# sunjay/portrayer

Hardware: AMD Instinct MI355X
Metric: Mray/s (primary+shadow+secondary) at 1920x1080 SAMPLES=64 (higher is better)
Workload: dtype f64; 1 GPU; big-scene (1000 analytic primitives, 3 point lights, reference scene script) 1920x1080 SAMPLES=64; width=1920, height=1080, samples=64, traversal=flat, sampling=counter-based jitter, seed 0, partition=single GPU, rays_per_frame=367740795

## Files before the change

### include/portrayer_hip.h

```cpp
#ifndef PORTRAYER_HIP_H
#define PORTRAYER_HIP_H

#include <stdint.h>

#ifdef __cplusplus
extern "C" {
#endif

#define PT_ABI_VERSION 8

enum { PT_PRIM_SPHERE = 0, PT_PRIM_TRIANGLE = 1, PT_PRIM_MESH = 2, PT_PRIM_KDMESH = 3, PT_PRIM_PLANE = 4, PT_PRIM_CUBE = 5, PT_PRIM_CYLINDER = 6, PT_PRIM_CONE = 7 };
enum { PT_TRAVERSE_FLAT = 1, PT_TRAVERSE_KD = 2, PT_TRAVERSE_HIER = 3 };
enum { PT_SAMPLE_CENTRE = 0, PT_SAMPLE_RNG = 1 };

enum {
    PT_OK = 0,
    PT_ERR_ARGUMENT = -1,
    PT_ERR_DEVICE = -2,
    PT_ERR_NO_SCENE = -3,
    PT_ERR_SLICE = -4,
    PT_ERR_SCENE = -5,
    PT_ERR_TRAVERSAL = -6
};

// ... 370 lines not shown
int pt_test_scene_info(const pt_context *ctx, uint64_t out[4]);
int pt_test_vertex_box_shape(const pt_context *ctx, uint64_t out[2]);
int pt_test_math(pt_context *ctx, int op, uint64_t n, const double *a, const double *b, double *out);
int pt_test_pow_host(uint64_t n, const double *x, const double *y, double *port, double *libm);
int pt_test_libm_host(int op, uint64_t n, const double *a, const double *b, double *out);
int pt_test_work_items(const pt_render_params *params, uint32_t *sample_count, uint64_t *sample_index_sum, uint32_t *chunk_length_sum,
                       uint64_t *n_items, uint32_t *lane_pixels_chunks_samples);
typedef struct pt_scene_traits {
    int32_t traverse;
    uint32_t n_nodes, n_lights;
    int32_t has_meshes;
    int32_t has_kdmesh;
    int32_t reflective;
    int32_t reflective_opaque;
    int32_t glossy;
    int32_t area_light;
    int32_t pad;
    uint64_t instanced_tris;
} pt_scene_traits;
int pt_test_kernel_choice(const pt_scene_traits *traits, int mode, int textured, uint32_t *kernel_mode, uint32_t *kernel_variant);
int pt_test_raypk(uint64_t n, int body, const double *origins, const double *directions, const double *t_max, const float *box_lo, const float *box_hi,
                  int32_t *verdict, float *t_near, float *t_far);
int pt_test_certain_shadow(uint64_t n, int type, const double *fwd, const double *inv, const double *P, const double *L, int32_t *out_certain, int32_t *out_exact_hit);
int pt_test_pixel_beam(uint64_t n, const double *cameras, const uint32_t *pixels, const double *jitters, const float *box_lo, const float *box_hi,
                       int32_t *accept, float *bound, int32_t *walk, double *rays);
int pt_test_pixel_list_summary(pt_context *ctx, uint64_t *out);
int pt_test_rect_beam(uint64_t n, const double *cameras, const uint32_t *rects, const double *offsets, const float *box_lo, const float *box_hi,
                      int32_t *accept, float *bound, int32_t *walk, double *rays);
int pt_test_pixel_list_records(pt_context *ctx, uint32_t *out, uint64_t words, uint64_t *info);
int pt_test_film_fold_host(uint32_t n, const double *samples, const uint32_t *cuts, uint32_t n_cuts, double out_sum[3]);
int pt_test_film_moments_host(uint32_t n, const double *samples, const uint32_t *cuts, uint32_t n_cuts, double out_sum[3], double *out_q, double *out_err);
int pt_test_film_plan_host(uint32_t width, uint32_t height, const pt_rect *slice, const uint32_t *budget, uint32_t max_samples, uint32_t round, uint32_t *list, uint32_t cap,
                           uint32_t *n_out);
int pt_test_film_plan(pt_context *ctx, uint32_t width, uint32_t height, const pt_rect *slice, const uint32_t *budget, uint32_t max_samples, uint32_t round, uint32_t *list, uint32_t cap,
                      uint32_t *n_out);
int pt_test_denoise_host(uint32_t width, uint32_t height, const pt_denoise_params *params, const double *linear, const double *variance, const uint32_t *counts,
                         const pt_denoise_guides *guides, double *out_linear, double *out_variance);
int pt_test_denoise_albedo_host(uint32_t width, uint32_t height, const pt_denoise_params *params, const double *linear, const double *variance, const uint32_t *counts,
                                const pt_denoise_guides *guides, const double *albedo, double *out_linear, double *out_variance);

#ifdef __cplusplus
}
#endif
#endif
```

### portrayer_amd/_hip.py

```python
from __future__ import annotations

import ctypes as C
import os
from typing import Optional

import numpy as np

PKG_DIR = os.path.dirname(os.path.abspath(__file__))
LIB_PATH = os.path.join(PKG_DIR, "libportrayer_hip.so")

TRAVERSE_FLAT, TRAVERSE_KD, TRAVERSE_HIER = 1, 2, 3
SAMPLE_CENTRE, SAMPLE_RNG = 0, 1
OK, ERR_ARGUMENT, ERR_DEVICE, ERR_NO_SCENE, ERR_SLICE, ERR_SCENE, ERR_TRAVERSAL = 0, -1, -2, -3, -4, -5, -6
KERNEL_WAVES_MASK, KERNEL_INTERPRETER, KERNEL_PARK, KERNEL_COUNTING, KERNEL_TEXTURED, KERNEL_FORK, KERNEL_CHAIN = 15, 16, 32, 64, 128, 256, 512

_dp = C.POINTER(C.c_double)
_ip = C.POINTER(C.c_int32)
_up = C.POINTER(C.c_uint32)
_u64p = C.POINTER(C.c_uint64)
_u8p = C.POINTER(C.c_uint8)


class PortrayerHipError(RuntimeError):
    pass
# ... 173 lines not shown

class PtStats(C.Structure):
    _fields_ = [(n, C.c_uint64) for n in ("primary", "shadow", "reflect", "refract", "depth11_skipped", "hits", "n_inner", "n_leaf",
                                          "n_analytic", "n_tri", "n_bbox", "kd_plane_miss", "stack_overflow")] + \
               [("kernel_ms", C.c_double), ("total_ms", C.c_double), ("diag", C.c_uint64 * 8), ("kernel_mode", C.c_uint32), ("kernel_variant", C.c_uint32)]

    def as_dict(self):
        d = {n: (float if n.endswith("_ms") else int)(getattr(self, n)) for n, _ in self._fields_ if n != "diag"}
        d["diag"] = [int(x) for x in self.diag]
        return d


_lib: Optional[C.CDLL] = None

EXPORTS = ["pt_abi_version", "pt_device_count", "pt_context_create", "pt_context_destroy", "pt_last_error", "pt_scene_upload",
           "pt_render", "pt_render_device", "pt_render_finish", "pt_context_stream", "pt_context_next_slot", "pt_compact_bytes", "pt_untile_device", "pt_tile_slot_pixel", "pt_untile_host", "pt_device_alloc",
           "pt_device_free", "pt_copy_to_device", "pt_copy_from_device", "pt_synchronize", "pt_measure_copy_bandwidth", "pt_test_cast_rays",
           "pt_test_math", "pt_test_work_items", "pt_node_create", "pt_node_destroy", "pt_node_last_error", "pt_node_ranks", "pt_node_uses_rccl", "pt_node_context",
           "pt_node_scene_upload", "pt_node_render", "pt_node_upload_background", "pt_node_render_resident", "pt_node_download_image",
           "pt_node_device", "pt_node_frame_begin", "pt_node_frame_end", "pt_node_frames_in_flight", "pt_node_last_frame_host_ms", "pt_node_last_frame_rank_kernel_ms", "pt_test_pow_host", "pt_test_libm_host",
           "pt_aov", "pt_aov_device", "pt_aov_finish", "pt_rays", "pt_rays_device", "pt_rays_finish", "pt_segments", "pt_segments_device",
           "pt_radiance", "pt_radiance_device", "pt_radiance_finish", "pt_scene_update", "pt_node_scene_update", "pt_scene_deform", "pt_node_scene_deform", "pt_scene_mesh_rebuildable", "pt_test_scene_bytes", "pt_test_scene_info",
           "pt_vertex_bounds_device", "pt_scene_deform_device", "pt_test_vertex_box_shape", "pt_test_raypk", "pt_test_certain_shadow", "pt_test_pixel_beam", "pt_test_pixel_list_summary", "pt_test_rect_beam", "pt_test_pixel_list_records",
           "pt_film_create", "pt_film_destroy", "pt_film_reset", "pt_film_add", "pt_film_add_device", "pt_film_resolve", "pt_film_resolve_device", "pt_film_counts",
           "pt_test_film_fold_host",
           "pt_film_create_moments", "pt_film_add_map", "pt_film_add_map_device", "pt_film_error", "pt_film_error_device", "pt_film_budget_device",
           "pt_test_film_moments_host", "pt_test_film_plan_host", "pt_test_film_plan",
           "pt_film_denoise", "pt_film_denoise_device", "pt_test_denoise_host",
           "pt_guides", "pt_guides_device", "pt_guides_finish", "pt_film_denoise_albedo", "pt_film_denoise_albedo_device", "pt_test_denoise_albedo_host",
           "pt_ao", "pt_ao_device", "pt_ao_finish", "pt_test_ao_rays_host", "pt_test_ao_tables",
           "pt_gather", "pt_gather_device", "pt_gather_finish", "pt_test_kernel_choice",
           "pt_chart_triangles", "pt_chart", "pt_chart_device", "pt_test_chart_host",
           "pt_direct", "pt_direct_device", "pt_direct_finish", "pt_test_direct_host"]


def header_functions():
    import re
    with open(os.path.join(os.path.dirname(os.path.dirname(os.path.abspath(__file__))), "include", "portrayer_hip.h")) as fh:
        text = re.sub(r"/\*.*?\*/", "", fh.read(), flags=re.S)
    return sorted(set(re.findall(r"\b(pt_[a-z0-9_]+)\s*\(", text)))


def missing_symbols():
    l = lib()
    return [n for n in header_functions() if not hasattr(l, n)]

# ... 50 lines not shown
        l.pt_untile_device.argtypes = [C.c_void_p, C.POINTER(PtRenderParams), C.c_void_p, C.c_void_p, C.c_void_p]
        l.pt_tile_slot_pixel.restype = C.c_int
        l.pt_tile_slot_pixel.argtypes = [C.POINTER(PtRenderParams), C.c_uint32, C.c_uint32, _up, _up]
        l.pt_untile_host.restype = C.c_int
        l.pt_untile_host.argtypes = [C.POINTER(PtRenderParams), _u8p, _u8p]
        l.pt_device_alloc.restype = C.c_int
        l.pt_device_alloc.argtypes = [C.c_void_p, C.c_uint64, C.POINTER(C.c_void_p)]
        l.pt_device_free.restype = C.c_int
        l.pt_device_free.argtypes = [C.c_void_p, C.c_void_p]
        l.pt_copy_to_device.restype = C.c_int
        l.pt_copy_to_device.argtypes = [C.c_void_p, C.c_void_p, C.c_void_p, C.c_uint64]
        l.pt_copy_from_device.restype = C.c_int
        l.pt_copy_from_device.argtypes = [C.c_void_p, C.c_void_p, C.c_void_p, C.c_uint64]
        l.pt_synchronize.restype = C.c_int
        l.pt_synchronize.argtypes = [C.c_void_p]
        l.pt_measure_copy_bandwidth.restype = C.c_int
        l.pt_measure_copy_bandwidth.argtypes = [C.c_void_p, C.c_uint64, C.c_int, _dp]
        l.pt_test_cast_rays.restype = C.c_int
        l.pt_test_cast_rays.argtypes = [C.c_void_p, C.c_uint64, _dp, _dp, C.c_int, _dp, _ip, _ip]
        l.pt_test_work_items.restype = C.c_int
        l.pt_test_work_items.argtypes = [C.c_void_p, C.POINTER(C.c_uint32), C.POINTER(C.c_uint64), C.POINTER(C.c_uint32), C.POINTER(C.c_uint64), C.POINTER(C.c_uint32)]
        l.pt_test_certain_shadow.restype = C.c_int
        l.pt_test_certain_shadow.argtypes = [C.c_uint64, C.c_int, _dp, _dp, _dp, _dp, _ip, _ip]
        l.pt_test_raypk.restype = C.c_int
        l.pt_test_raypk.argtypes = [C.c_uint64, C.c_int, _dp, _dp, _dp, C.POINTER(C.c_float), C.POINTER(C.c_float), _ip, C.POINTER(C.c_float), C.POINTER(C.c_float)]
        l.pt_test_pixel_list_summary.restype = C.c_int
        l.pt_test_pixel_list_summary.argtypes = [C.c_void_p, C.POINTER(C.c_uint64)]
        l.pt_test_pixel_beam.restype = C.c_int
        l.pt_test_pixel_beam.argtypes = [C.c_uint64, _dp, C.POINTER(C.c_uint32), _dp, C.POINTER(C.c_float), C.POINTER(C.c_float), _ip, C.POINTER(C.c_float), _ip, _dp]
        l.pt_test_rect_beam.restype = C.c_int
        l.pt_test_rect_beam.argtypes = l.pt_test_pixel_beam.argtypes
        l.pt_test_pixel_list_records.restype = C.c_int
        l.pt_test_pixel_list_records.argtypes = [C.c_void_p, C.POINTER(C.c_uint32), C.c_uint64, C.POINTER(C.c_uint64)]
        l.pt_test_math.restype = C.c_int
        l.pt_test_math.argtypes = [C.c_void_p, C.c_int, C.c_uint64, _dp, _dp, _dp]
        l.pt_node_create.restype = C.c_int
        l.pt_node_create.argtypes = [C.c_int, _ip, C.POINTER(C.c_void_p)]
        l.pt_node_destroy.restype = None
        l.pt_node_destroy.argtypes = [C.c_void_p]
        l.pt_node_last_error.restype = C.c_char_p
        l.pt_node_last_error.argtypes = [C.c_void_p]
        l.pt_node_ranks.restype = C.c_int
        l.pt_node_ranks.argtypes = [C.c_void_p]
        l.pt_node_uses_rccl.restype = C.c_int
        l.pt_node_uses_rccl.argtypes = [C.c_void_p]
        l.pt_node_context.restype = C.c_void_p
# ... 215 lines not shown
```

### portrayer_amd/csrc/pt_api.hip

```cpp
#include <type_traits>

#include "pt_context.h"
#include "pt_aov_inst.h"
#include "pt_guides_inst.h"
#include "pt_chart.h"
#include "pt_rays_inst.h"
#include "pt_segments_inst.h"
#include "pt_ao_inst.h"
#include "pt_direct_inst.h"
#include "pt_radiance_inst.h"
#include "pt_gather_inst.h"
#include "pt_film_inst.h"
#include "pt_film_map_inst.h"
#include "pt_denoise.h"
#include "pt_render_inst.h"
#include "pt_shade.h"
#include "pt_pixel_list.h"

template <int MODE>
__global__ void __launch_bounds__(PT_BLOCK) pt_cast_kernel(PtSceneView sc, uint64_t n, const double* o, const double* d, int any,
                                                          double* out_t, int32_t* out_node, int32_t* out_sub, unsigned int* overflow) {
    extern __shared__ uint32_t pt_lds[];
    PtStack stk;
    stk.base = pt_lds + threadIdx.x;
// ... 87 lines not shown
__global__ void __launch_bounds__(256) pt_occ_seed_kernel(uint32_t* __restrict__ occ, uint32_t n, int hashed, uint64_t seed, uint32_t all, uint32_t n_nodes) {
    const uint32_t i = blockIdx.x * blockDim.x + threadIdx.x;
    if (i >= n) return;
    occ[i] = hashed ? (uint32_t)(pt_rng_key(seed, i) % ((uint64_t)n_nodes + 1u)) : all + 1u;
}

__global__ void __launch_bounds__(256) pt_eye_table_kernel(const double* __restrict__ inv, double* __restrict__ tab, uint32_t n_nodes, double ex, double ey, double ez) {
    const uint32_t i = blockIdx.x * blockDim.x + threadIdx.x;
    if (i >= n_nodes) return;
    const double* m = inv + 12 * (size_t)i;
    double* o = tab + 12 * (size_t)i;
    const PtVec3 e = pt_xform_point(m, pt_v3(ex, ey, ez));
    o[0] = m[0]; o[1] = m[1]; o[2] = m[2]; o[3] = e.x;
    o[4] = m[4]; o[5] = m[5]; o[6] = m[6]; o[7] = e.y;
    o[8] = m[8]; o[9] = m[9]; o[10] = m[10]; o[11] = e.z;
}

__global__ void __launch_bounds__(256) pt_certain_table_kernel(const uint32_t* __restrict__ info, const double* __restrict__ fwd, const double* __restrict__ inv, float* __restrict__ tab,
                                                               uint32_t n_nodes) {
    const uint32_t i = blockIdx.x * blockDim.x + threadIdx.x;
    if (i >= n_nodes) return;
    pt_certain_ball(info[4 * (size_t)i], fwd + 12 * (size_t)i, inv + 12 * (size_t)i, tab + 4 * (size_t)i);
}

#ifndef PT_PL_DEPTH_FIRST
#define PT_PL_BLOCK 64
#define PT_PL_PENDING 1024u
#define PT_PL_STEP_CANDS 128u
#define PT_PL_CANDS 128u
#define PT_PL_WAVE_SYNC() do { __builtin_amdgcn_fence(__ATOMIC_RELEASE, "wavefront"); __builtin_amdgcn_wave_barrier(); __builtin_amdgcn_fence(__ATOMIC_ACQUIRE, "wavefront"); } while (0)
static __device__ __forceinline__ float pt_pl_scalar(float v) { return __builtin_bit_cast(float, __builtin_amdgcn_readfirstlane(__builtin_bit_cast(int, v))); }
static __device__ __forceinline__ uint32_t pt_pl_lanes_below(unsigned long long m) { return __builtin_amdgcn_mbcnt_hi((uint32_t)(m >> 32), __builtin_amdgcn_mbcnt_lo((uint32_t)m, 0u)); }
__global__ void __launch_bounds__(PT_PL_BLOCK) pt_pixel_list_kernel(PtRenderArgs a, uint32_t* __restrict__ table, uint32_t cap, uint32_t pend_cap) {
    __shared__ uint32_t s_list[PT_PL_BLOCK / 64][PT_PL_K][64];
    __shared__ uint32_t s_pend[PT_PL_BLOCK / 64][PT_PL_PENDING];
    __shared__ uint4 s_cand[PT_PL_BLOCK / 64][PT_PL_CANDS * 2u];
    static_assert(PT_PL_CANDS >= PT_PL_STEP_CANDS, "the empty buffer takes a step's candidates");
    const uint32_t wave = threadIdx.x >> 6, lane = threadIdx.x & 63u;
    const uint32_t tile_local = PT_UNIFORM_U32(blockIdx.x * (PT_PL_BLOCK / 64) + wave);
    if (tile_local >= a.n_slots / 64u) return;
    const PtSceneView& sc = a.scene;
    const uint32_t slot = tile_local * 64u + lane;
    uint32_t x, y, tx, ty;
    pt_slot_to_pixel(a, slot, &x, &y);
    pt_slot_to_pixel(a, tile_local * 64u, &tx, &ty);
    const PtBeam beam = pt_beam_setup(a.cam, (double)x, (double)y);
// ... 552 lines not shown
    PT_HIP(c, hipMemcpy(out, (const char*)sl.eye_tab.p + c->pl_off, need * 4, hipMemcpyDeviceToHost));
    return PT_OK;
}

extern "C" int pt_test_certain_shadow(uint64_t n, int type, const double* fwd, const double* inv, const double* P, const double* L, int32_t* out_certain, int32_t* out_exact_hit) {
    if (!fwd || !inv || !P || !L || !out_certain || !out_exact_hit || type < 0 || type > 7) return PT_ERR_ARGUMENT;
    for (uint64_t i = 0; i < n; i++) {
        float ball[4];
        pt_certain_ball((uint32_t)type, fwd + 12 * i, inv + 12 * i, ball);
        const PtVec3 p = pt_v3(P[3 * i], P[3 * i + 1], P[3 * i + 2]), l = pt_v3(L[3 * i], L[3 * i + 1], L[3 * i + 2]);
        out_certain[i] = ball[3] > 0.0f && pt_certain_lane(ball, (float)p.x, (float)p.y, (float)p.z, (float)l.x, (float)l.y, (float)l.z) ? 1 : 0;
        PtRay r;
        r.o = p;
        const PtVec3 hit_to_light = l - p;
        r.d = hit_to_light / pt_length(hit_to_light);
        const PtRay local = pt_ray_to_local(inv + 12 * i, r);
        double t;
        uint32_t part = 0;
        out_exact_hit[i] = pt_unit_prim_hit((uint32_t)type, local, PT_EPSILON, INFINITY, &t, &part) ? 1 : 0;
    }
    return PT_OK;
}

static bool pt_kd_semantics(int mode) { return mode == PT_MODE_KD || mode == PT_MODE_KD_NOMESH || mode == PT_MODE_KD_MESH; }
static int pt_stack_lds_cap(const PtSceneView& sc, size_t block_budget, size_t frame_bytes) {
    int lds_cap = block_budget > frame_bytes ? (int)((block_budget - frame_bytes) / (PT_BLOCK * 4)) : 0;
    lds_cap = std::max(lds_cap, 2);
    if (const char* e = getenv("PORTRAYER_LDS_STACK")) lds_cap = std::max(1, atoi(e));
    int cap = std::min(lds_cap, sc.stack_cap);
    if (pt_kd_semantics(sc.mode)) cap = std::max(cap, (sc.stack_cap + 63) / 64 + 2);
    return cap;
}
static size_t pt_stack_column(const PtSceneView& sc, int stack_lds_cap) {
    const int wave_rows = std::min(std::max(8, (sc.stack_cap + 63) / 64), std::max(stack_lds_cap, 8));
    const int stack_spill_entries = std::max(sc.stack_cap - stack_lds_cap + wave_rows, 0);
    return (size_t)std::max(stack_spill_entries, sc.stack_cap);
}

static void pt_walk_sizing(PtRenderArgs& r, int waves) {
    r.stack_lds_cap = pt_stack_lds_cap(r.scene, waves == 3 ? 52 * 1024 : 39 * 1024, 0);
    r.grid_share = 1;
}
struct PtInterp { bool tex, park; };
static PtInterp pt_interp_sizing(const pt_context* c, PtRenderArgs& r) {
    PtInterp k;
    k.tex = r.scene.mat_maps != nullptr;
// ... 120 lines not shown
    if ((rc = pt_reserve(c, sl.spill, spill_bytes))) return rc;
    const size_t stack_column = pt_stack_column(a.scene, a.stack_lds_cap);
    if ((rc = pt_reserve(c, sl.stack_spill, (size_t)a.n_lanes * stack_column * 4))) return rc;
    const size_t misc_head = 256 + sizeof(PtCounters) + PT_FINE_QUEUES * PT_QUEUE_STRIDE * 4;
    size_t occ_bytes = (size_t)(a.n_slots / 64) * a.scene.n_lights * 4;
    if (!(a.scene.mode == PT_MODE_FLAT_NOMESH || a.scene.mode == PT_MODE_HIER_NOMESH) || occ_bytes > ((size_t)4 << 20)) occ_bytes = 0;
    if (const char* e = getenv("PORTRAYER_SHADOW_CACHE")) if (atoi(e) <= 0) occ_bytes = 0;
    bool occ_seed = false, occ_hashed = false;
    uint64_t occ_seed_value = 0;
    uint32_t occ_all = 0;
    if (const char* e = getenv("PORTRAYER_OCC_SEED"); e && *e && occ_bytes) {
        char* end = nullptr;
        if (strncmp(e, "all:", 4) == 0) {
            const unsigned long long k = strtoull(e + 4, &end, 10);
            if (end == e + 4 || *end || k >= a.scene.n_nodes) return pt_fail(c, PT_ERR_ARGUMENT, std::string("PORTRAYER_OCC_SEED=") + e + ": K must be a node index below " + std::to_string(a.scene.n_nodes));
            occ_all = (uint32_t)k;
        } else {
            occ_seed_value = strtoull(e, &end, 10);
            if (end == e || *end) return pt_fail(c, PT_ERR_ARGUMENT, std::string("PORTRAYER_OCC_SEED=") + e + ": expected all:<node> or a decimal seed");
            occ_hashed = true;
        }
        occ_seed = true;
    }
    if ((rc = pt_reserve(c, sl.misc, misc_head + occ_bytes))) return rc;
    if ((rc = pt_reserve(c, sl.accum, (size_t)a.n_slots * a.n_chunks * 3 * sizeof(double)))) return rc;
    a.accum = (double*)sl.accum.p;
#ifndef PT_NO_EYE_TABLE
    const bool eye_table = a.scene.mode == PT_MODE_FLAT_NOMESH && a.scene.n_nodes > 0;
#else
    const bool eye_table = false;
#endif
#ifndef PT_NO_CERTAIN_SHADOW
    const bool certain_table = a.scene.mode == PT_MODE_FLAT_NOMESH && a.scene.n_nodes > 0 && occ_bytes != 0;
#else
    const bool certain_table = false;
#endif
#ifndef PT_NO_PIXEL_LISTS
    const bool list_header = eye_table;
#ifdef PT_PIXEL_LIST_STATS
    const bool list_reader = true;
#else
    const bool list_reader = !stats;
#endif
    bool pixel_lists = eye_table && list_reader && (a.run_variant == PT_RUN_LINE3 || a.run_variant == PT_RUN_LINE4 || a.run_variant == PT_RUN_LINE5) && a.k_log2 + a.c_log2 == 6u &&
                       a.scene.n_nodes <= PT_PL_MAX_NODES && a.n_slots != 0;
    if (const char* e = getenv("PORTRAYER_PIXEL_LISTS")) if (atoi(e) <= 0) pixel_lists = false;
    uint32_t list_cap = PT_PL_K;
// ... 6 lines not shown
    uint32_t list_pending = 1024u;
    if (const char* e = getenv("PORTRAYER_PIXEL_LIST_PENDING"); e && *e) {
        char* end = nullptr;
        const unsigned long long k = strtoull(e, &end, 10);
        if (end == e || *end || k < 1u || k > list_pending) return pt_fail(c, PT_ERR_ARGUMENT, std::string("PORTRAYER_PIXEL_LIST_PENDING=") + e + ": expected 1 .. " + std::to_string(list_pending));
        list_pending = (uint32_t)k;
    }
#else
    const bool list_header = false, pixel_lists = false;
    const uint32_t list_cap = 0, list_pending = 0;
#endif
    const size_t list_off = pt_pl_header_offset((uint32_t)a.scene.n_nodes);
    a.eye_tab = nullptr;
    if (eye_table || certain_table) {
        if ((rc = pt_reserve(c, sl.eye_tab, list_header ? list_off + pt_pl_bytes(pixel_lists ? a.n_slots : 0u) : (size_t)a.scene.n_nodes * (12 * sizeof(double) + 4 * sizeof(float))))) return rc;
        a.eye_tab = (const double*)sl.eye_tab.p;
    }
    a.spill = (double*)sl.spill.p;
    a.stack_spill = (uint32_t*)sl.stack_spill.p;
    a.work_counter = (unsigned int*)sl.misc.p;
    a.overflow_flag = (unsigned int*)sl.misc.p + 1;
    a.counters = (PtCounters*)((char*)sl.misc.p + 256);
    a.work_queues = (unsigned int*)((char*)sl.misc.p + 256 + sizeof(PtCounters));
    a.occluders = occ_bytes ? (uint32_t*)((char*)sl.misc.p + misc_head) : nullptr;
    a.occ_row = std::max<uint32_t>(a.div_tiles_x.d / std::max<uint32_t>(a.tile_ranks, 1u), 1u);
    c->last_mode = (uint32_t)a.scene.mode;
    c->last_variant = pt_choice_variant(choice, tex) | (stats ? PT_KERNEL_COUNTING : 0u);
    PT_HIP(c, hipMemsetAsync(sl.misc.p, 0, misc_head + occ_bytes, stream));
    if (occ_seed) {
        const uint32_t n_occ = (uint32_t)(occ_bytes / 4);
        hipLaunchKernelGGL(pt_occ_seed_kernel, dim3((n_occ + 255) / 256), dim3(256), 0, stream, a.occluders, n_occ, occ_hashed ? 1 : 0, occ_seed_value, occ_all, a.scene.n_nodes);
        PT_HIP(c, hipGetLastError());
        if (getenv("PORTRAYER_VERBOSE")) fprintf(stderr, "[pt_render] occluder table: %u entries seeded (PORTRAYER_OCC_SEED=%s)\n", n_occ, getenv("PORTRAYER_OCC_SEED"));
    }
    sl.mode = c->last_mode; sl.variant = c->last_variant; sl.counted = stats;
    PT_HIP(c, hipEventRecord(sl.ev0, stream));
    if (a.n_items) {
        if (eye_table) {
            hipLaunchKernelGGL(pt_eye_table_kernel, dim3((a.scene.n_nodes + 255) / 256), dim3(256), 0, stream, a.scene.inv, (double*)sl.eye_tab.p, (uint32_t)a.scene.n_nodes,
                               a.cam.eye[0], a.cam.eye[1], a.cam.eye[2]);
            PT_HIP(c, hipGetLastError());
        }
        if (certain_table) {
            hipLaunchKernelGGL(pt_certain_table_kernel, dim3((a.scene.n_nodes + 255) / 256), dim3(256), 0, stream, a.scene.info, a.scene.fwd, a.scene.inv, (float*)((double*)sl.eye_tab.p + 12 * (size_t)a.scene.n_nodes),
                               (uint32_t)a.scene.n_nodes);
            PT_HIP(c, hipGetLastError());
        }
        if (list_header) {
            uint32_t* const header = (uint32_t*)((char*)sl.eye_tab.p + list_off);
            PT_HIP(c, hipMemsetD32Async((hipDeviceptr_t)header, pixel_lists ? 1 : 0, 16, stream));
            if (pixel_lists) {
                const uint32_t tiles = a.n_slots / 64u;
                hipLaunchKernelGGL(pt_pixel_list_kernel, dim3((tiles + PT_PL_BLOCK / 64 - 1) / (PT_PL_BLOCK / 64)), dim3(PT_PL_BLOCK), 0, stream, a, header + 16, list_cap, list_pending);
                PT_HIP(c, hipGetLastError());
            }
        }
        c->pl_slot = pixel_lists ? slot_index : -1; c->pl_slots = a.n_slots; c->pl_off = list_off + 64; c->pl_nodes = (uint32_t)a.scene.n_nodes;
        PT_HIP(c, pt_dispatch(a, stats, c->n_cu, stream, &grid, true));
        hipLaunchKernelGGL(pt_finish_kernel, dim3((a.n_slots + PT_BLOCK - 1) / PT_BLOCK), dim3(PT_BLOCK), 0, stream, a);
        PT_HIP(c, hipGetLastError());
    }
    PT_HIP(c, hipEventRecord(sl.ev1, stream));
    PT_HIP(c, hipMemcpyAsync(sl.host, sl.misc.p, stats ? PT_SLOT_BYTES : 8, hipMemcpyDeviceToHost, stream));
    PT_HIP(c, hipEventRecord(sl.copy_done, stream));
    return PT_OK;
}

static int pt_collect_stats(pt_context* c, pt_stats* st, int slot_index) {
    pt_context::Slot& sl = c->slot[slot_index];
    if (st) memset(st, 0, sizeof *st);
// ... 1601 lines not shown
```

### portrayer_amd/csrc/pt_certain.h

```cpp
#pragma once

#include "pt_prims.h"

#define PT_CERTAIN_S_MAX 4.0f
#define PT_CERTAIN_REACH2_LOG2 24
#define PT_CERTAIN_WW_MIN 1e-30f

PT_HD void pt_certain_ball(uint32_t type, const double* fwd, const double* inv, float* out) {
    out[0] = out[1] = out[2] = out[3] = 0.0f;
    double rm;
    if (type == PT_SPHERE) rm = 1.0;
    else if (type == PT_CUBE) rm = 0.5;
    else return;
    const PtVec3 cm = pt_v3(0.0, 0.0, 0.0);
    const PtVec3 c = pt_xform_point(fwd, cm);
    const PtVec3 back = pt_xform_point(inv, c) - cm;
    const double e = fabs(back.x) + fabs(back.y) + fabs(back.z);
    double g = 0.0, h = 0.0;
    for (int i = 0; i < 3; i++) {
        double gi = 0.0, hi = 0.0;
        for (int j = 0; j < 3; j++) {
            gi += fabs(inv[4 * i] * inv[4 * j] + inv[4 * i + 1] * inv[4 * j + 1] + inv[4 * i + 2] * inv[4 * j + 2]);
            hi += fabs(fwd[4 * i] * fwd[4 * j] + fwd[4 * i + 1] * fwd[4 * j + 1] + fwd[4 * i + 2] * fwd[4 * j + 2]);
        }
// ... 18 lines not shown
#if defined(__HIP_DEVICE_COMPILE__)
    float f;
    asm volatile("v_cvt_f32_f64 %0, %1" : "=v"(f) : "v"(x));
    return f;
#else
    return (float)x;
#endif
}

PT_HD bool pt_certain_lane(const float* rec, float px, float py, float pz, float lx, float ly, float lz) {
    const float vx = rec[0] - px, vy = rec[1] - py, vz = rec[2] - pz;
    const float wx = lx - px, wy = ly - py, wz = lz - pz;
    const float ww = __builtin_fmaf(wz, wz, __builtin_fmaf(wy, wy, wx * wx));
    const float vw = __builtin_fmaf(vz, wz, __builtin_fmaf(vy, wy, vx * wx));
#if defined(__HIP_DEVICE_COMPILE__)
    const float s = vw * __builtin_amdgcn_rcpf(ww);
#else
    const float s = vw / ww;
#endif
    const float ux = __builtin_fmaf(-s, wx, vx), uy = __builtin_fmaf(-s, wy, vy), uz = __builtin_fmaf(-s, wz, vz);
    const float uu = __builtin_fmaf(uz, uz, __builtin_fmaf(uy, uy, ux * ux));
    return (vw > 0.0f) & (ww > PT_CERTAIN_WW_MIN) & (s < PT_CERTAIN_S_MAX) & (uu < rec[3]) & (__builtin_ldexpf(s * vw, -PT_CERTAIN_REACH2_LOG2) < rec[3]);
}
```

### portrayer_amd/csrc/pt_context.h

```cpp
#pragma once
#include <hip/hip_runtime.h>

#include <algorithm>
#include <chrono>
#include <cmath>
#include <cstdio>
#include <cstring>
#include <string>
#include <vector>

#include "../../include/portrayer_hip.h"
#include "pt_build.h"
#include "pt_bvh.h"
#include "pt_shade.h"

struct PtBuf {
    void* p = nullptr;
    size_t bytes = 0;
    PtBuf() = default;
    PtBuf(const PtBuf&) = delete;
    PtBuf& operator=(const PtBuf&) = delete;
    ~PtBuf() { if (p) hipFree(p); }
};

// ... 38 lines not shown
    uint32_t launch_seq = 0;
    PtSceneView view;
    bool have_scene = false;
    struct Slot {
        PtBuf spill, stack_spill, accum, misc;
        PtBuf eye_tab;
        hipStream_t stream = nullptr;
        hipEvent_t ev0 = nullptr, ev1 = nullptr;
        hipEvent_t copy_done = nullptr;
        unsigned char* host = nullptr;
        bool pending = false, counted = false;
        uint32_t mode = 0, variant = 0;
        std::chrono::steady_clock::time_point t_start;
    };
    static constexpr int PT_SLOTS = 2;
    Slot slot[PT_SLOTS];
    int slot_next = 0;
    int slot_oldest = 0;
    uint32_t last_mode = 0, last_variant = 0;
    int pl_slot = -1;
    uint32_t pl_slots = 0;
    size_t pl_off = 0;
    uint32_t pl_nodes = 0;
    struct Aov {
        PtPass pass;
        PtBuf out[6];
        PtBuf albedo;
        bool guides = false;
        PtBuf chart_owner, chart_uv, chart_covered;
        bool chart = false;
    } aov;
    struct Rays {
        PtPass pass;
        PtBuf in[2], in_t_max, out[7];
        PtRaySort sort;
    } rays;
    struct Radiance {
        PtPass pass;
        PtBuf in[3], out;
        PtRaySort sort;
    } radiance;
    PtPass* const passes[3] = {&aov.pass, &rays.pass, &radiance.pass};
    std::vector<pt_film*> films;
    pt_film* film_open = nullptr;
    struct Resident {
        int traverse = 0;
// ... 72 lines not shown
```

### portrayer_amd/csrc/pt_render_simple.h

```cpp
#pragma once

#include "pt_shade.h"

#if !defined(PT_NO_CERTAIN_SHADOW) && (!defined(PT_INST_MODE) || PT_INST_MODE == 3)
#define PT_CERTAIN_SHADOW_FORM 1
#endif

#if !defined(PT_NO_PIXEL_LISTS) && !defined(PT_NO_EYE_TABLE) && (!defined(PT_INST_MODE) || PT_INST_MODE == 3)
#define PT_PIXEL_LIST_FORM 1
#include "pt_pixel_list.h"
typedef uint32_t pt_u32x2 __attribute__((ext_vector_type(2)));
PT_HD uint32_t pt_sload1(const void* p) {
#if defined(__HIP_DEVICE_COMPILE__)
    uint32_t v;
    asm volatile("s_load_dword %0, %1, 0x0\n\ts_waitcnt lgkmcnt(0)" : "=s"(v) : "s"(pt_uniform_ptr(p)) : "memory");
    return v;
#else
    return *static_cast<const uint32_t*>(p);
#endif
}
PT_HD pt_u32x2 pt_sload2(const void* p) {
    pt_u32x2 v;
#if defined(__HIP_DEVICE_COMPILE__)
    asm volatile("s_load_dwordx2 %0, %1, 0x0\n\ts_waitcnt lgkmcnt(0)" : "=s"(v) : "s"(pt_uniform_ptr(p)) : "memory");
// ... 396 lines not shown
                constexpr bool OCC = !CHAIN && (MODE == PT_MODE_FLAT_NOMESH || MODE == PT_MODE_HIER_NOMESH);
#else
                constexpr bool OCC = !STATS && !CHAIN && (MODE == PT_MODE_FLAT_NOMESH || MODE == PT_MODE_HIER_NOMESH);
#endif
                if (OCC && a.occluders) {
                    const uint32_t tile_local = pt_fastdiv(w >> (a.k_log2 + a.c_log2), a.div_groups);
                    occ.entry = a.occluders + (size_t)tile_local * sc.n_lights + li;
                    occ.back = tile_local >= a.occ_row ? a.occ_row * sc.n_lights : 0u;
                }
#else
                double light_dist = 0.0;
                if (shaded && area) {
                    PtItemLane it;
                    uint32_t x2, y2;
                    pt_item_lane_fast(a, w, lane, &it, &x2, &y2);
                    const uint64_t key = pt_rng_key(a.seed, (uint64_t)y * a.width + x);
                    const uint32_t d0 = CHAIN ? draw : udraw;
                    double a_coord = 2.0 * pt_rng_draw(key, it.sample, d0) - 1.0;
                    double b_coord = 2.0 * pt_rng_draw(key, it.sample, d0 + 1) - 1.0;
                    lpos = lpos + (aa * a_coord + ab * b_coord);
                    if (CHAIN) draw += 2;
                }
                if (area) udraw += 2;
                PtOccRef occ{nullptr, 0u, li};
#ifdef PT_OCCLUDER_STATS
                constexpr bool OCC = !CHAIN && (MODE == PT_MODE_FLAT_NOMESH || MODE == PT_MODE_HIER_NOMESH);
#else
                constexpr bool OCC = !STATS && !CHAIN && (MODE == PT_MODE_FLAT_NOMESH || MODE == PT_MODE_HIER_NOMESH);
#endif
                if (OCC && a.occluders) {
                    const uint32_t tile_local = pt_fastdiv(w >> (a.k_log2 + a.c_log2), a.div_groups);
                    occ.entry = a.occluders + (size_t)tile_local * sc.n_lights + li;
                    occ.back = tile_local >= a.occ_row ? a.occ_row * sc.n_lights : 0u;
                }
                constexpr bool CERTAIN = OCC && MODE == PT_MODE_FLAT_NOMESH;
                [[maybe_unused]] PtOccHint hint{0u, 0u, 0u, 0u};
                if (CERTAIN && occ.entry) {
                    const float* const certain_tab = (const float*)(a.eye_tab + 12 * (size_t)sc.n_nodes);
                    const uint32_t* const entry = (const uint32_t*)pt_uniform_ptr(occ.entry);
                    hint.own = PT_UNIFORM_U32(entry[0]);
                    hint.up = occ.back ? PT_UNIFORM_U32(entry[-(long)occ.back]) : 0u;
                    hint.loaded = 1u;
                    const uint32_t cand = hint.own ? hint.own : hint.up;
                    if (cand != 0u) {
                        const pt_u32x4 rec = pt_sload4(certain_tab + 4 * (size_t)(cand - 1u));
                        float ball[4];
#pragma unroll
                        for (int k = 0; k < 4; k++) ball[k] = __builtin_bit_cast(float, (uint32_t)rec[k]);
                        if (ball[3] > 0.0f) {
                            const float pf[3] = {pt_f32_here(sray.o.x), pt_f32_here(sray.o.y), pt_f32_here(sray.o.z)};
                            const float lx = (float)lpos.x, ly = (float)lpos.y, lz = (float)lpos.z;
                            const bool c1 = shaded && pt_certain_lane(ball, pf[0], pf[1], pf[2], lx, ly, lz);
                            const unsigned long long want = PT_BALLOT(shaded), got = PT_BALLOT(c1);
                            bool settled = want != 0ull && got == want;
                            if (settled) {
                                hint.certain = 3u;
                                if (!STATS && hint.own != cand && lane == (unsigned)(__ffsll((long long)__ballot(1)) - 1)) occ.entry[0] = cand;
                            }
#if PT_OCCLUDER_STATS + 0 == 2
                            else if (hint.own != 0u && hint.up != 0u && hint.up != hint.own) {
                                const pt_u32x4 rec2 = pt_sload4(certain_tab + 4 * (size_t)(hint.up - 1u));
                                float ball2[4];
#pragma unroll
                                for (int k = 0; k < 4; k++) ball2[k] = __builtin_bit_cast(float, (uint32_t)rec2[k]);
                                if (ball2[3] > 0.0f) {
                                    const bool c2 = shaded && !c1 && pt_certain_lane(ball2, pf[0], pf[1], pf[2], lx, ly, lz);
                                    settled = want != 0ull && (got | PT_BALLOT(c2)) == want;
                                    if (settled) hint.certain = 2u;
                                }
                            }
#endif
                            if (!STATS && settled) { PT_SEC_END(6); continue; }
                        }
                    }
                }
                if (shaded) {
                    PtVec3 hit_to_light = lpos - sray.o;
                    light_dist = pt_length(hit_to_light);
                    sray.d = hit_to_light / light_dist;
                    fr.l(PT_L_TAG) = light_dist;
                    if (STATS) cnt.shadow++;
                }
                PtHit sh;
                sh.t = INFINITY; sh.node = PT_NO_HIT; sh.sub = 0;
                PT_SEC_END(6);
#endif
#if defined(PT_CERTAIN_SHADOW_FORM) && !defined(PT_CYCLES) && !defined(PT_ABLATE)
                if (CERTAIN && occ.entry) {
                    const int words = a.stack_lds_cap * 64;
                    pt_trace_packet_occ<STATS, false>(sc, sray, shaded, sh, pt_lds + (size_t)(threadIdx.x >> 6) * words, words, a.overflow_flag, &cnt, occ, hint);
                } else
#endif
                pt_trace_wave<MODE, STATS>(a, sray, shaded, true, sh, stk, pt_lds, &cnt, occ);
                PT_SEC_SKIP();
// ... 93 lines not shown
```

### portrayer_amd/csrc/pt_walk_wave.h

```cpp
#pragma once

typedef uint32_t pt_u32x16 __attribute__((ext_vector_type(16)));
typedef uint32_t pt_u32x8 __attribute__((ext_vector_type(8)));
typedef uint32_t pt_u32x4 __attribute__((ext_vector_type(4)));
PT_HD const void* pt_uniform_ptr(const void* p) {
#if defined(__HIP_DEVICE_COMPILE__)
    const unsigned long long a = (unsigned long long)p;
    const unsigned long long lo = (uint32_t)__builtin_amdgcn_readfirstlane((int)(uint32_t)a), hi = (uint32_t)__builtin_amdgcn_readfirstlane((int)(uint32_t)(a >> 32));
    return (const void*)((hi << 32) | lo);
#else
    return p;
#endif
}
PT_HD pt_u32x8 pt_sload8(const void* p) {
    pt_u32x8 v;
#if defined(__HIP_DEVICE_COMPILE__)
    asm volatile("s_load_dwordx8 %0, %1, 0x0\n\ts_waitcnt lgkmcnt(0)" : "=s"(v) : "s"(pt_uniform_ptr(p)) : "memory");
#else
    v = *static_cast<const pt_u32x8*>(p);
#endif
    return v;
}
PT_HD pt_u32x4 pt_sload4(const void* p) {
    pt_u32x4 v;
// ... 609 lines not shown
    if (has_ray) { best.t = INFINITY; best.node = PT_NO_HIT; best.sub = 0; }
    if (cand != 0u && has_ray) {
        const bool identity_ok = HIER && pt_ray_identity_safe(ray, has_ray);
        PtHit probe = best;
        blocked = pt_test_node_uniform<false, HIER>(sc, cand - 1u, ray, identity_ok, probe, cnt);
        if (!STATS && blocked) best = probe;
    }
    const unsigned long long blocked_mask = PT_BALLOT(blocked);
    const uint32_t first = (uint32_t)__ffsll((long long)__ballot(1)) - 1u;
    if (!STATS && blocked_mask != 0ull && blocked_mask == rays) {
        if (own != cand && PT_LANE_ID() == first) entry[0] = cand;
        return;
    }
    if (STATS) pt_trace_packet_walk<STATS, HIER>(sc, ray, has_ray, any, best, wstack, wwords, overflow, cnt);
    else pt_trace_packet_walk<STATS, HIER>(sc, ray, has_ray, any, best, wstack, wwords, overflow, cnt, !blocked);
    const unsigned long long hit_mask = PT_BALLOT(has_ray && best.node != PT_NO_HIT);
    const uint32_t now = hit_mask ? (uint32_t)__builtin_amdgcn_readlane((int)best.node, (int)(__ffsll((long long)hit_mask) - 1)) + 1u : 0u;
    if (rays && now != own && PT_LANE_ID() == first) entry[0] = now;
    if (COUNT_OCC && rays && occ.light < 3u && PT_LANE_ID() == first) {
        cnt->diag[2 * occ.light] += 1ull | (hit_mask ? 1ull << 32 : 0ull);
        if (hit_mask == rays) cnt->diag[2 * occ.light + 1] += 1ull | (blocked_mask == rays ? 1ull << 32 : 0ull);
#if PT_OCCLUDER_STATS + 0 == 2
        if (hit_mask == rays && blocked_mask == rays && (hint.certain & 1u)) cnt->diag[6] += 1ull << (21 * occ.light);
        if (hit_mask == rays && (hint.certain & 2u)) cnt->diag[7] += 1ull << (21 * occ.light);
#else
        if (cand) cnt->diag[6] += 1ull | (own ? 1ull << 32 : 0ull);
        if (blocked_mask) cnt->diag[7]++;
#endif
    }
#else
    pt_trace_packet_walk<STATS, HIER>(sc, ray, has_ray, any, best, wstack, wwords, overflow, cnt);
#endif
}

template <bool STATS, bool HIER, bool EYE = false>
PT_HD void pt_trace_packet(const PtSceneView& sc, const PtRay& ray, bool has_ray, bool any, PtHit& best, uint32_t* wstack, int wwords,
                           unsigned int* overflow, PtCounters* cnt, PtOccRef occ = PtOccRef{nullptr, 0u, 0u}, const double* eye_tab = nullptr) {
    if (EYE) {
        pt_trace_packet_walk<STATS, HIER, EYE>(sc, ray, has_ray, false, best, wstack, wwords, overflow, cnt, true, eye_tab);
        return;
    }
#if defined(__HIP_DEVICE_COMPILE__)
#ifdef PT_OCCLUDER_STATS
    constexpr bool COUNT_OCC = STATS;
#else
    constexpr bool COUNT_OCC = false;
#endif
// ... 216 lines not shown
```

### profiles/occluder_stats.py

```python
#!/usr/bin/env python3
import os, shutil, sys, tempfile, json
ROOT = os.path.dirname(os.path.dirname(os.path.abspath(__file__)))
tmp = tempfile.mkdtemp()
shutil.copytree(os.path.join(ROOT, "portrayer_amd"), os.path.join(tmp, "portrayer_amd"), ignore=shutil.ignore_patterns("csrc", "host"))
shutil.copy(os.path.join(sys.argv[1], "libportrayer_hip.so"), os.path.join(tmp, "portrayer_amd", "libportrayer_hip.so"))
sys.path.insert(0, tmp)
sys.path.insert(1, os.path.join(ROOT, "tests"))
from portrayer_amd import _hip as H, host
from scene_dsl import ASSETS, default_background
mode = sys.argv[2]
sc = host.Scene.example("big-scene", assets=ASSETS)
r = host.Renderer(sc, H.TRAVERSE_HIER if mode == "hier" else H.TRAVERSE_FLAT)
w, h = 1920, 1080
_, _, st = r.render(sc.camera, w, h, default_background(w, h), samples=64, seed=0, sample_mode=H.SAMPLE_RNG, stats=True, want_linear=False)
r.close()
d = st["diag"]
lo = lambda x: x & 0xFFFFFFFF
hi = lambda x: x >> 32
out = {"mode": mode, "shadow_rays": st["shadow"], "n_inner": st["n_inner"], "primary": st["primary"], "lights": []}
for l in range(3):
    out["lights"].append({"walks": lo(d[2 * l]), "some_lane_occluded": hi(d[2 * l]), "all_occluded": lo(d[2 * l + 1]), "candidate_ends": hi(d[2 * l + 1])})
if len(sys.argv) > 3 and sys.argv[3] == "certain":
    for l in range(3):
        assert out["lights"][l]["walks"] < (1 << 21), "a 21-bit field would overflow"
        out["lights"][l]["candidate_ends_and_its_ball_settles"] = (d[6] >> (21 * l)) & 0x1FFFFF
        out["lights"][l]["all_occluded_and_two_balls_settle"] = (d[7] >> (21 * l)) & 0x1FFFFF
else:
    out["walks_with_candidate"] = lo(d[6]); out["candidate_from_own_tile"] = hi(d[6]); out["candidate_blocked_a_lane"] = d[7]
print("OCCSTATS " + json.dumps(out), flush=True)
```

Measured before the change: 63930 Mray/s.

## Skip shadow walks for point lights enclosed inside an opaque primitive

Adds a per-frame kernel that checks each point light against every primitive's inscribed certainty ball. For each light that sits inside a ball it records the enclosing node and a conservative reach radius. In the flat no-mesh shading loop, a wave skips its shadow traversal when every shaded lane's hit point lies within that radius, treating the light as fully occluded. This removes BVH/flat walks toward lights sealed inside solid geometry, at the cost of one small extra launch, one scalar load per light and per-lane distance checks. Correctness depends on the conservative ball bounds; statistics hooks are added to verify no unblocked lane is ever settled.

```diff
diff --git a/include/portrayer_hip.h b/include/portrayer_hip.h
--- a/include/portrayer_hip.h
+++ b/include/portrayer_hip.h
@@ -416,6 +416,9 @@
 int pt_test_raypk(uint64_t n, int body, const double *origins, const double *directions, const double *t_max, const float *box_lo, const float *box_hi,
                   int32_t *verdict, float *t_near, float *t_far);
 int pt_test_certain_shadow(uint64_t n, int type, const double *fwd, const double *inv, const double *P, const double *L, int32_t *out_certain, int32_t *out_exact_hit);
+int pt_test_dark_light(uint64_t n, int type, const double *fwd, const double *inv, const double *P, const double *L, const double *area, int32_t *out_flagged, int32_t *out_guard,
+                       int32_t *out_exact_hit);
+int pt_test_dark_lights(pt_context *ctx, uint32_t *out, uint64_t words, uint64_t *info);
 int pt_test_pixel_beam(uint64_t n, const double *cameras, const uint32_t *pixels, const double *jitters, const float *box_lo, const float *box_hi,
                        int32_t *accept, float *bound, int32_t *walk, double *rays);
 int pt_test_pixel_list_summary(pt_context *ctx, uint64_t *out);
diff --git a/portrayer_amd/_hip.py b/portrayer_amd/_hip.py
--- a/portrayer_amd/_hip.py
+++ b/portrayer_amd/_hip.py
@@ -219,6 +219,7 @@
            "pt_aov", "pt_aov_device", "pt_aov_finish", "pt_rays", "pt_rays_device", "pt_rays_finish", "pt_segments", "pt_segments_device",
            "pt_radiance", "pt_radiance_device", "pt_radiance_finish", "pt_scene_update", "pt_node_scene_update", "pt_scene_deform", "pt_node_scene_deform", "pt_scene_mesh_rebuildable", "pt_test_scene_bytes", "pt_test_scene_info",
            "pt_vertex_bounds_device", "pt_scene_deform_device", "pt_test_vertex_box_shape", "pt_test_raypk", "pt_test_certain_shadow", "pt_test_pixel_beam", "pt_test_pixel_list_summary", "pt_test_rect_beam", "pt_test_pixel_list_records",
+           "pt_test_dark_light", "pt_test_dark_lights",
            "pt_film_create", "pt_film_destroy", "pt_film_reset", "pt_film_add", "pt_film_add_device", "pt_film_resolve", "pt_film_resolve_device", "pt_film_counts",
            "pt_test_film_fold_host",
            "pt_film_create_moments", "pt_film_add_map", "pt_film_add_map_device", "pt_film_error", "pt_film_error_device", "pt_film_budget_device",
@@ -315,6 +316,10 @@
         l.pt_test_work_items.argtypes = [C.c_void_p, C.POINTER(C.c_uint32), C.POINTER(C.c_uint64), C.POINTER(C.c_uint32), C.POINTER(C.c_uint64), C.POINTER(C.c_uint32)]
         l.pt_test_certain_shadow.restype = C.c_int
         l.pt_test_certain_shadow.argtypes = [C.c_uint64, C.c_int, _dp, _dp, _dp, _dp, _ip, _ip]
+        l.pt_test_dark_light.restype = C.c_int
+        l.pt_test_dark_light.argtypes = [C.c_uint64, C.c_int, _dp, _dp, _dp, _dp, _dp, _ip, _ip, _ip]
+        l.pt_test_dark_lights.restype = C.c_int
+        l.pt_test_dark_lights.argtypes = [C.c_void_p, C.POINTER(C.c_uint32), C.c_uint64, C.POINTER(C.c_uint64)]
         l.pt_test_raypk.restype = C.c_int
         l.pt_test_raypk.argtypes = [C.c_uint64, C.c_int, _dp, _dp, _dp, C.POINTER(C.c_float), C.POINTER(C.c_float), _ip, C.POINTER(C.c_float), C.POINTER(C.c_float)]
         l.pt_test_pixel_list_summary.restype = C.c_int
diff --git a/portrayer_amd/csrc/pt_api.hip b/portrayer_amd/csrc/pt_api.hip
--- a/portrayer_amd/csrc/pt_api.hip
+++ b/portrayer_amd/csrc/pt_api.hip
@@ -133,6 +133,26 @@
     if (i >= n_nodes) return;
     pt_certain_ball(info[4 * (size_t)i], fwd + 12 * (size_t)i, inv + 12 * (size_t)i, tab + 4 * (size_t)i);
 }
+
+#ifndef PT_NO_DARK_LIGHTS
+__global__ void __launch_bounds__(256) pt_dark_light_kernel(const double* __restrict__ lights, const float* __restrict__ balls, uint32_t* __restrict__ words, uint32_t n_nodes) {
+    __shared__ uint32_t best;
+    const double* const light = lights + 15 * (size_t)blockIdx.x;
+    if (threadIdx.x == 0) best = 0xFFFFFFFFu;
+    __syncthreads();
+    float rec[4];
+    for (uint32_t i = threadIdx.x; i < n_nodes; i += blockDim.x)
+        if (pt_dark_light(light, balls + 4 * (size_t)i, rec)) atomicMin(&best, i);
+    __syncthreads();
+    if (threadIdx.x != 0) return;
+    uint32_t* const o = words + PT_DARK_WORDS * (size_t)blockIdx.x;
+    const bool found = best != 0xFFFFFFFFu && pt_dark_light(light, balls + 4 * (size_t)best, rec);
+    for (int k = 0; k < 4; k++) o[k] = found ? __builtin_bit_cast(uint32_t, rec[k]) : 0u;
+    o[4] = found ? best + 1u : 0u;
+    o[5] = found ? __builtin_bit_cast(uint32_t, PT_DARK_D2_MIN) : 0u;
+    o[6] = o[7] = 0u;
+}
+#endif
 
 #ifndef PT_PL_DEPTH_FIRST
 #define PT_PL_BLOCK 64
@@ -731,6 +751,51 @@
     return PT_OK;
 }
 
+extern "C" int pt_test_dark_light(uint64_t n, int type, const double* fwd, const double* inv, const double* P, const double* L, const double* area, int32_t* out_flagged,
+                                  int32_t* out_guard, int32_t* out_exact_hit) {
+    if (!fwd || !inv || !P || !L || !out_flagged || !out_guard || !out_exact_hit || type < 0 || type > 7) return PT_ERR_ARGUMENT;
+    for (uint64_t i = 0; i < n; i++) {
+        float ball[4], rec[4];
+        pt_certain_ball((uint32_t)type, fwd + 12 * i, inv + 12 * i, ball);
+        double light[15];
+        for (int k = 0; k < 15; k++) light[k] = 0.0;
+        for (int k = 0; k < 3; k++) light[k] = L[3 * i + k];
+        if (area) for (int k = 0; k < 6; k++) light[9 + k] = area[6 * i + k];
+        const PtVec3 p = pt_v3(P[3 * i], P[3 * i + 1], P[3 * i + 2]), l = pt_v3(light[0], light[1], light[2]);
+#ifndef PT_NO_DARK_LIGHTS
+        out_flagged[i] = pt_dark_light(light, ball, rec) ? 1 : 0;
+        out_guard[i] = out_flagged[i] && pt_dark_lane(rec, (float)p.x, (float)p.y, (float)p.z) ? 1 : 0;
+#else
+        (void)rec;
+        out_flagged[i] = out_guard[i] = 0;
+#endif
+        PtRay r;
+        r.o = p;
+        const PtVec3 hit_to_light = l - p;
+        r.d = hit_to_light / pt_length(hit_to_light);
+        const PtRay local = pt_ray_to_local(inv + 12 * i, r);
+        double t;
+        uint32_t part = 0;
+        out_exact_hit[i] = pt_unit_prim_hit((uint32_t)type, local, PT_EPSILON, INFINITY, &t, &part) ? 1 : 0;
+    }
+    return PT_OK;
+}
+
+extern "C" int pt_test_dark_lights(pt_context* c, uint32_t* out, uint64_t words, uint64_t* info) {
+    if (!c || !info) return PT_ERR_ARGUMENT;
+    info[0] = 0; info[1] = PT_DARK_WORDS;
+    if (c->dark_slot < 0 || c->dark_lights == 0) return PT_OK;
+    info[0] = c->dark_lights;
+    const size_t need = (size_t)c->dark_lights * PT_DARK_WORDS;
+    if (!out || words < need) return PT_OK;
+    PT_HIP(c, hipSetDevice(c->device));
+    PT_HIP(c, hipDeviceSynchronize());
+    const pt_context::Slot& sl = c->slot[c->dark_slot];
+    if (sl.misc.bytes < c->dark_off + need * 4) return pt_fail(c, PT_ERR_ARGUMENT, "the slot's buffer no longer holds that launch's records");
+    PT_HIP(c, hipMemcpy(out, (const char*)sl.misc.p + c->dark_off, need * 4, hipMemcpyDeviceToHost));
+    return PT_OK;
+}
+
 static bool pt_kd_semantics(int mode) { return mode == PT_MODE_KD || mode == PT_MODE_KD_NOMESH || mode == PT_MODE_KD_MESH; }
 static int pt_stack_lds_cap(const PtSceneView& sc, size_t block_budget, size_t frame_bytes) {
     int lds_cap = block_budget > frame_bytes ? (int)((block_budget - frame_bytes) / (PT_BLOCK * 4)) : 0;
@@ -897,7 +962,15 @@
         }
         occ_seed = true;
     }
-    if ((rc = pt_reserve(c, sl.misc, misc_head + occ_bytes))) return rc;
+#ifndef PT_NO_DARK_LIGHTS
+    const size_t dark_bytes = (a.scene.mode == PT_MODE_FLAT_NOMESH && occ_bytes != 0) ? (size_t)a.scene.n_lights * PT_DARK_WORDS * 4 : 0;
+    bool dark_lights = dark_bytes != 0 && a.scene.n_nodes > 0;
+    if (const char* e = getenv("PORTRAYER_DARK_LIGHTS")) if (atoi(e) <= 0) dark_lights = false;
+#else
+    const size_t dark_bytes = 0;
+    const bool dark_lights = false;
+#endif
+    if ((rc = pt_reserve(c, sl.misc, misc_head + dark_bytes + occ_bytes))) return rc;
     if ((rc = pt_reserve(c, sl.accum, (size_t)a.n_slots * a.n_chunks * 3 * sizeof(double)))) return rc;
     a.accum = (double*)sl.accum.p;
 #ifndef PT_NO_EYE_TABLE
@@ -950,11 +1023,11 @@
     a.overflow_flag = (unsigned int*)sl.misc.p + 1;
     a.counters = (PtCounters*)((char*)sl.misc.p + 256);
     a.work_queues = (unsigned int*)((char*)sl.misc.p + 256 + sizeof(PtCounters));
-    a.occluders = occ_bytes ? (uint32_t*)((char*)sl.misc.p + misc_head) : nullptr;
+    a.occluders = occ_bytes ? (uint32_t*)((char*)sl.misc.p + misc_head + dark_bytes) : nullptr;
     a.occ_row = std::max<uint32_t>(a.div_tiles_x.d / std::max<uint32_t>(a.tile_ranks, 1u), 1u);
     c->last_mode = (uint32_t)a.scene.mode;
     c->last_variant = pt_choice_variant(choice, tex) | (stats ? PT_KERNEL_COUNTING : 0u);
-    PT_HIP(c, hipMemsetAsync(sl.misc.p, 0, misc_head + occ_bytes, stream));
+    PT_HIP(c, hipMemsetAsync(sl.misc.p, 0, misc_head + dark_bytes + occ_bytes, stream));
     if (occ_seed) {
         const uint32_t n_occ = (uint32_t)(occ_bytes / 4);
         hipLaunchKernelGGL(pt_occ_seed_kernel, dim3((n_occ + 255) / 256), dim3(256), 0, stream, a.occluders, n_occ, occ_hashed ? 1 : 0, occ_seed_value, occ_all, a.scene.n_nodes);
@@ -974,6 +1047,14 @@
                                (uint32_t)a.scene.n_nodes);
             PT_HIP(c, hipGetLastError());
         }
+#ifndef PT_NO_DARK_LIGHTS
+        if (certain_table && dark_lights) {
+            hipLaunchKernelGGL(pt_dark_light_kernel, dim3((uint32_t)a.scene.n_lights), dim3(256), 0, stream, a.scene.lights, (const float*)((const double*)sl.eye_tab.p + 12 * (size_t)a.scene.n_nodes),
+                               (uint32_t*)((char*)sl.misc.p + misc_head), (uint32_t)a.scene.n_nodes);
+            PT_HIP(c, hipGetLastError());
+        }
+        c->dark_slot = dark_bytes ? slot_index : -1; c->dark_lights = (uint32_t)a.scene.n_lights; c->dark_off = misc_head;
+#endif
         if (list_header) {
             uint32_t* const header = (uint32_t*)((char*)sl.eye_tab.p + list_off);
             PT_HIP(c, hipMemsetD32Async((hipDeviceptr_t)header, pixel_lists ? 1 : 0, 16, stream));
diff --git a/portrayer_amd/csrc/pt_certain.h b/portrayer_amd/csrc/pt_certain.h
--- a/portrayer_amd/csrc/pt_certain.h
+++ b/portrayer_amd/csrc/pt_certain.h
@@ -64,3 +64,31 @@
     const float uu = __builtin_fmaf(uz, uz, __builtin_fmaf(uy, uy, ux * ux));
     return (vw > 0.0f) & (ww > PT_CERTAIN_WW_MIN) & (s < PT_CERTAIN_S_MAX) & (uu < rec[3]) & (__builtin_ldexpf(s * vw, -PT_CERTAIN_REACH2_LOG2) < rec[3]);
 }
+
+#define PT_DARK_D2_MIN 1e-30f
+#define PT_DARK_WORDS 8
+
+PT_HD bool pt_dark_light(const double* light, const float* ball, float* out) {
+    out[0] = out[1] = out[2] = out[3] = 0.0f;
+    const bool area = !((light[9] == 0.0 && light[10] == 0.0 && light[11] == 0.0) || (light[12] == 0.0 && light[13] == 0.0 && light[14] == 0.0));
+    if (area) return false;
+    const double rho2 = (double)ball[3];
+    if (!(rho2 > 0.0)) return false;
+    const PtVec3 l = pt_v3(light[0], light[1], light[2]);
+    const PtVec3 d = l - pt_v3((double)ball[0], (double)ball[1], (double)ball[2]);
+    if (!(pt_dot(d, d) <= rho2 * ((1.0 - 0x1p-6) * (1.0 - 0x1p-6) * (1.0 - 0x1p-40)))) return false;
+    const double reach = sqrt(rho2) * (4096.0 * (1.0 - 0x1p-10)) - 0x1p-21 * sqrt(pt_dot(l, l));
+    if (!(reach > 0.0)) return false;
+    const double ceil2 = reach * reach;
+    if (!(ceil2 > 1e-30 && ceil2 < 1e37)) return false;
+    float f = (float)ceil2;
+    if ((double)f > ceil2) f = __builtin_bit_cast(float, __builtin_bit_cast(uint32_t, f) - 1u);
+    out[0] = (float)l.x; out[1] = (float)l.y; out[2] = (float)l.z; out[3] = f;
+    return true;
+}
+
+PT_HD bool pt_dark_lane(const float* rec, float px, float py, float pz) {
+    const float wx = rec[0] - px, wy = rec[1] - py, wz = rec[2] - pz;
+    const float d2 = __builtin_fmaf(wz, wz, __builtin_fmaf(wy, wy, wx * wx));
+    return (d2 >= PT_DARK_D2_MIN) & (d2 <= rec[3]);
+}
diff --git a/portrayer_amd/csrc/pt_context.h b/portrayer_amd/csrc/pt_context.h
--- a/portrayer_amd/csrc/pt_context.h
+++ b/portrayer_amd/csrc/pt_context.h
@@ -84,6 +84,9 @@
     uint32_t pl_slots = 0;
     size_t pl_off = 0;
     uint32_t pl_nodes = 0;
+    int dark_slot = -1;
+    uint32_t dark_lights = 0;
+    size_t dark_off = 0;
     struct Aov {
         PtPass pass;
         PtBuf out[6];
diff --git a/portrayer_amd/csrc/pt_render_simple.h b/portrayer_amd/csrc/pt_render_simple.h
--- a/portrayer_amd/csrc/pt_render_simple.h
+++ b/portrayer_amd/csrc/pt_render_simple.h
@@ -442,19 +442,34 @@
                     if (CHAIN) draw += 2;
                 }
                 if (area) udraw += 2;
-                PtOccRef occ{nullptr, 0u, li};
 #ifdef PT_OCCLUDER_STATS
                 constexpr bool OCC = !CHAIN && (MODE == PT_MODE_FLAT_NOMESH || MODE == PT_MODE_HIER_NOMESH);
 #else
                 constexpr bool OCC = !STATS && !CHAIN && (MODE == PT_MODE_FLAT_NOMESH || MODE == PT_MODE_HIER_NOMESH);
 #endif
+                [[maybe_unused]] bool dark = false;
+#if !defined(PT_NO_DARK_LIGHTS)
+                if (OCC && MODE == PT_MODE_FLAT_NOMESH && a.occluders) {
+                    const pt_u32x4 dk = pt_sload4(a.occluders - PT_DARK_WORDS * (size_t)(sc.n_lights - li));
+                    if (dk[3] != 0u) {
+                        float drec[4];
+#pragma unroll
+                        for (int k = 0; k < 4; k++) drec[k] = __builtin_bit_cast(float, (uint32_t)dk[k]);
+                        const bool g = shaded & pt_dark_lane(drec, pt_f32_here(sray.o.x), pt_f32_here(sray.o.y), pt_f32_here(sray.o.z));
+                        const unsigned long long want = PT_BALLOT(shaded);
+                        dark = want != 0ull && PT_BALLOT(g) == want;
+                        if (!STATS && dark) { PT_SEC_END(6); continue; }
+                    }
+                }
+#endif
+                PtOccRef occ{nullptr, 0u, li};
                 if (OCC && a.occluders) {
                     const uint32_t tile_local = pt_fastdiv(w >> (a.k_log2 + a.c_log2), a.div_groups);
                     occ.entry = a.occluders + (size_t)tile_local * sc.n_lights + li;
                     occ.back = tile_local >= a.occ_row ? a.occ_row * sc.n_lights : 0u;
                 }
                 constexpr bool CERTAIN = OCC && MODE == PT_MODE_FLAT_NOMESH;
-                [[maybe_unused]] PtOccHint hint{0u, 0u, 0u, 0u};
+                [[maybe_unused]] PtOccHint hint{0u, 0u, 0u, (STATS && dark) ? 4u : 0u};
                 if (CERTAIN && occ.entry) {
                     const float* const certain_tab = (const float*)(a.eye_tab + 12 * (size_t)sc.n_nodes);
                     const uint32_t* const entry = (const uint32_t*)pt_uniform_ptr(occ.entry);
@@ -474,22 +489,9 @@
                             const unsigned long long want = PT_BALLOT(shaded), got = PT_BALLOT(c1);
                             bool settled = want != 0ull && got == want;
                             if (settled) {
-                                hint.certain = 3u;
+                                hint.certain |= 3u;
                                 if (!STATS && hint.own != cand && lane == (unsigned)(__ffsll((long long)__ballot(1)) - 1)) occ.entry[0] = cand;
                             }
-#if PT_OCCLUDER_STATS + 0 == 2
-                            else if (hint.own != 0u && hint.up != 0u && hint.up != hint.own) {
-                                const pt_u32x4 rec2 = pt_sload4(certain_tab + 4 * (size_t)(hint.up - 1u));
-                                float ball2[4];
-#pragma unroll
-                                for (int k = 0; k < 4; k++) ball2[k] = __builtin_bit_cast(float, (uint32_t)rec2[k]);
-                                if (ball2[3] > 0.0f) {
-                                    const bool c2 = shaded && !c1 && pt_certain_lane(ball2, pf[0], pf[1], pf[2], lx, ly, lz);
-                                    settled = want != 0ull && (got | PT_BALLOT(c2)) == want;
-                                    if (settled) hint.certain = 2u;
-                                }
-                            }
-#endif
                             if (!STATS && settled) { PT_SEC_END(6); continue; }
                         }
                     }
diff --git a/portrayer_amd/csrc/pt_walk_wave.h b/portrayer_amd/csrc/pt_walk_wave.h
--- a/portrayer_amd/csrc/pt_walk_wave.h
+++ b/portrayer_amd/csrc/pt_walk_wave.h
@@ -655,7 +655,10 @@
         if (hit_mask == rays) cnt->diag[2 * occ.light + 1] += 1ull | (blocked_mask == rays ? 1ull << 32 : 0ull);
 #if PT_OCCLUDER_STATS + 0 == 2
         if (hit_mask == rays && blocked_mask == rays && (hint.certain & 1u)) cnt->diag[6] += 1ull << (21 * occ.light);
-        if (hit_mask == rays && (hint.certain & 2u)) cnt->diag[7] += 1ull << (21 * occ.light);
+        if (hint.certain & 4u) {
+            if (hit_mask == rays) cnt->diag[7] += 1ull << (21 * occ.light);
+            else cnt->kd_plane_miss++;
+        }
 #else
         if (cand) cnt->diag[6] += 1ull | (own ? 1ull << 32 : 0ull);
         if (blocked_mask) cnt->diag[7]++;
diff --git a/profiles/occluder_stats.py b/profiles/occluder_stats.py
--- a/profiles/occluder_stats.py
+++ b/profiles/occluder_stats.py
@@ -1,5 +1,5 @@
 #!/usr/bin/env python3
-import os, shutil, sys, tempfile, json
+import ctypes, os, shutil, sys, tempfile, json
 ROOT = os.path.dirname(os.path.dirname(os.path.abspath(__file__)))
 tmp = tempfile.mkdtemp()
 shutil.copytree(os.path.join(ROOT, "portrayer_amd"), os.path.join(tmp, "portrayer_amd"), ignore=shutil.ignore_patterns("csrc", "host"))
@@ -13,6 +13,13 @@
 r = host.Renderer(sc, H.TRAVERSE_HIER if mode == "hier" else H.TRAVERSE_FLAT)
 w, h = 1920, 1080
 _, _, st = r.render(sc.camera, w, h, default_background(w, h), samples=64, seed=0, sample_mode=H.SAMPLE_RNG, stats=True, want_linear=False)
+dark_nodes = None
+if len(sys.argv) > 3 and sys.argv[3] == "certain":
+    info = (ctypes.c_uint64 * 2)()
+    assert H.lib().pt_test_dark_lights(r.context, None, 0, info) == 0 and info[0] == 3 and info[1] == 8
+    words = (ctypes.c_uint32 * 24)()
+    assert H.lib().pt_test_dark_lights(r.context, words, 24, info) == 0
+    dark_nodes = [int(words[8 * l + 4]) - 1 for l in range(3)]
 r.close()
 d = st["diag"]
 lo = lambda x: x & 0xFFFFFFFF
@@ -24,7 +31,12 @@
     for l in range(3):
         assert out["lights"][l]["walks"] < (1 << 21), "a 21-bit field would overflow"
         out["lights"][l]["candidate_ends_and_its_ball_settles"] = (d[6] >> (21 * l)) & 0x1FFFFF
-        out["lights"][l]["all_occluded_and_two_balls_settle"] = (d[7] >> (21 * l)) & 0x1FFFFF
+        out["lights"][l]["dark_light_guard_settles"] = (d[7] >> (21 * l)) & 0x1FFFFF
+        out["lights"][l]["enclosed_in_node"] = dark_nodes[l]
+        assert out["lights"][l]["dark_light_guard_settles"] <= out["lights"][l]["all_occluded"]
+        assert dark_nodes[l] >= 0 or out["lights"][l]["dark_light_guard_settles"] == 0
+    out["settled_with_a_lane_unblocked"] = st["kd_plane_miss"]
+    assert st["kd_plane_miss"] == 0, "the dark-light guard settled a walk in which some lane is not blocked"
 else:
     out["walks_with_candidate"] = lo(d[6]); out["candidate_from_own_tile"] = hi(d[6]); out["candidate_blocked_a_lane"] = d[7]
 print("OCCSTATS " + json.dumps(out), flush=True)
```

After: 68760 Mray/s, median of 6. 1.08x the previous value.
